# rafifmalikdzaki/Multitask-Bonetumor-yolo

Measured on AMD Instinct MI355X. Metric: images/sec at 640x640 multitask fwd (det+seg+cls) + decode/NMS/masks, higher is better.
Workload: dtype bf16; 1 GPU; configs[1]: batch-16/GPU 640x640 multitask inference (ConvNeXt-T + C2f-BiFPN + Detect/Segment/cls) + decode + per-image NMS(top-100) + mask assembly; random-init weights; batch_per_gpu=16, img=640, parallelism=dp1 (batch sharded, no data-path collective)

## Files before the change

include/mtbt_hip.h:

```cpp
#ifndef MTBT_HIP_H
#define MTBT_HIP_H

#include <stdint.h>

#ifdef __cplusplus
extern "C" {
#endif

#define MTBT_OK 0
#define MTBT_EINVAL (-1)
#define MTBT_EALIGN (-2)
#define MTBT_ELAUNCH (-3)
#define MTBT_EWORKSPACE (-4)

#define MTBT_F32 0
#define MTBT_BF16 1
#define MTBT_F16 2

#define MTBT_ACT_NONE 0
#define MTBT_ACT_SILU 1
#define MTBT_ACT_ELU 2
#define MTBT_ACT_GELU 3
#define MTBT_ACT_DSILU 5
#define MTBT_ACT_DELU 6
// ... 39 lines not shown
  int64_t colsum_ws_bytes;
} mtbt_conv_args;

int mtbt_conv2d_nhwc(const mtbt_conv_args* a, void* stream);
int64_t mtbt_conv_colsum_workspace_bytes(int64_t pixels , int K, int with_squares);
int mtbt_conv_colsum_layout(const mtbt_conv_args* a, int64_t* rows, int32_t* pitch);
int mtbt_conv_kernel_choice(const mtbt_conv_args* a, int32_t* choice);

int mtbt_conv2d_nhwc_batch(const mtbt_conv_args* calls, int n, void* stream);
int mtbt_conv_batch_kernel_choice(const mtbt_conv_args* calls, int n, int32_t* choice);

int mtbt_stem_conv4x4_ln(const float* x, const float* w, const float* bias, const float* ln_w,
                         const float* ln_b, float ln_eps, void* y, int N, int H, int W, int Cout,
                         int out_dtype, void* stream);

int mtbt_dwconv_nhwc(const void* x, const void* w, const float* bias, const float* ln_w,
                     const float* ln_b, float ln_eps, const float* scale, const float* shift, int act,
                     void* y, int N, int H, int W, int C, int ksize, int dtype, void* stream);
int mtbt_dwconv3x3_mult_nhwc(const void* x, const void* w, const float* scale, const float* shift, int act, void* y,
                             int N, int H, int W, int C, int M, int dtype, void* stream);
int mtbt_dwconv_kernel_choice(int N, int H, int W, int C, int ksize, int ln, int act, int dtype, int32_t* choice);
int mtbt_dwconv3x3_mult_kernel_choice(int N, int H, int W, int C, int M, int act, int dtype, int32_t* choice);

int mtbt_layernorm_nhwc(const void* x, const float* w, const float* b, float eps, void* y,
                        int64_t pixels, int C, int dtype, void* stream);

typedef struct mtbt_fuse_args {
  const void* x[3];
  float wgt[3];
  int32_t resample[3];
// ... 691 lines not shown
```

multitask_bonetumor_yolo_amd/_lib.py:

```python
import ctypes as C
import os

_HERE = os.path.dirname(os.path.abspath(__file__))
LIB_PATH = os.path.join(_HERE, "csrc", "libmtbt_hip.so")

ABI_VERSION = 5
F32, BF16, F16 = 0, 1, 2
ACT_NONE, ACT_SILU, ACT_ELU, ACT_GELU, ACT_GELU_POLY, ACT_DSILU, ACT_DELU, ACT_DGELU, ACT_DGELU_POLY = 0, 1, 2, 3, 4, 5, 6, 7, 8
OUT_NHWC, OUT_CONVT2X2 = 0, 1
RES_ID, RES_UP_BILINEAR, RES_DOWN_MEAN, RES_UP_NEAREST, RES_MAXPOOL = 0, 1, 2, 3, 4
CONFUSION_MAX_NC = 64
WARP_CHUNK = 32
WARP_LIN_MAX, WARP_OFF_MAX = 1 << 26, 1 << 47
COPY_PASTE_CHUNK = 8
COPY_PASTE_MAX_ENTRIES = 16

ERRORS = {-1: "MTBT_EINVAL (bad argument / unsupported shape)", -2: "MTBT_EALIGN (misaligned pointer or stride)",
          -3: "MTBT_ELAUNCH (kernel launch failed)", -4: "MTBT_EWORKSPACE (workspace too small)"}


class ConvArgs(C.Structure):
    _fields_ = [
        ("x", C.c_void_p), ("w", C.c_void_p), ("y", C.c_void_p), ("scale", C.c_void_p), ("shift", C.c_void_p),
        ("res", C.c_void_p),
# ... 448 lines not shown
```

multitask_bonetumor_yolo_amd/csrc/dwconv.hip:

```cpp
#include "common.h"
#include "dwconv_args.h"

static int dw_dispatch(const DwArgs& a, int dtype, hipStream_t s) {
  if (dtype == MTBT_BF16) return mtbt_dw_run_bf16(a, s);
  if (dtype == MTBT_F16) return mtbt_dw_run_f16(a, s);
  if (dtype == MTBT_F32) return mtbt_dw_run_f32(a, s);
  return MTBT_EINVAL;
}

static int dw_check_shape(int N, int H, int W, int C, int ksize, int act) {
  if (N <= 0 || H <= 0 || W <= 0 || C <= 0 || C % 8 || C > 768) return MTBT_EINVAL;
  if (ksize != 3 && ksize != 7) return MTBT_EINVAL;
  if (act < 0 || act > MTBT_ACT_DGELU_POLY) return MTBT_EINVAL;
  if ((long)(W + 64) * C * 4 >= 0x7fff0000L || (long)H * W * C >= 0x7fff0000L) return MTBT_EINVAL;
  return MTBT_OK;
}

static int dw_dispatch_mult(const DwArgs& a, int Cx, int dtype, hipStream_t s) {
  if (dtype == MTBT_BF16) return mtbt_dw_run_mult_bf16(a, Cx, s);
  if (dtype == MTBT_F16) return mtbt_dw_run_mult_f16(a, Cx, s);
  if (dtype == MTBT_F32) return mtbt_dw_run_mult_f32(a, Cx, s);
  return MTBT_EINVAL;
}

static int dw_check_shape_mult(int N, int H, int W, int C, int M, int act) {
  if (N <= 0 || H <= 0 || W <= 0 || C <= 0 || C % 128 || (M != 1 && M != 2) || M * C > 768) return MTBT_EINVAL;
  if (act < 0 || act > MTBT_ACT_DGELU_POLY) return MTBT_EINVAL;
  if ((long)(W + 64) * M * C * 4 >= 0x7fff0000L || (long)H * W * M * C >= 0x7fff0000L) return MTBT_EINVAL;
  return MTBT_OK;
}

static int dwconv_entry(const void* x, const void* w, const float* bias, const float* ln_w, const float* ln_b, float ln_eps, const float* scale,
                        const float* shift, int act, void* y, void* raw, const void* res, int N, int H, int W, int C, int ksize, int dtype,
                        void* stream) {
  if (!x || !w || !y) return MTBT_EINVAL;
  if (int rc = dw_check_shape(N, H, W, C, ksize, act)) return rc;
  const bool ln = ln_w != nullptr;
  if (ln && (!ln_b || !bias || res)) return MTBT_EINVAL;
  if (!ln && (!scale || !shift || raw)) return MTBT_EINVAL;
  if (!aligned16(x) || !aligned16(y) || !aligned16(w) || (raw && !aligned16(raw)) || (res && !aligned16(res))) return MTBT_EALIGN;
  DwArgs a{x, w, bias, ln_w, ln_b, ln_eps, scale, shift, act, y, raw, res, N, H, W, C, ksize, nullptr};
  return dw_dispatch(a, dtype, reinterpret_cast<hipStream_t>(stream));
}

extern "C" int mtbt_dwconv_kernel_choice(int N, int H, int W, int C, int ksize, int ln, int act, int dtype, int32_t* choice) {
  if (!choice) return MTBT_EINVAL;
  if (int rc = dw_check_shape(N, H, W, C, ksize, act)) return rc;
  static const float some = 0.f;
  DwArgs a{nullptr, nullptr, nullptr, ln ? &some : nullptr, nullptr, 0.f, nullptr, nullptr, act, nullptr, nullptr, nullptr, N, H, W, C, ksize, choice};
  return dw_dispatch(a, dtype, nullptr);
}

extern "C" int mtbt_dwconv_nhwc(const void* x, const void* w, const float* bias, const float* ln_w, const float* ln_b,
                                float ln_eps, const float* scale, const float* shift, int act, void* y, int N, int H,
                                int W, int C, int ksize, int dtype, void* stream) {
  return dwconv_entry(x, w, bias, ln_w, ln_b, ln_eps, scale, shift, act, y, nullptr, nullptr, N, H, W, C, ksize, dtype, stream);
}

extern "C" int mtbt_dwconv_nhwc_train(const void* x, const void* w, const float* bias, const float* ln_w, const float* ln_b,
                                      float ln_eps, const float* scale, const float* shift, int act, void* y, void* raw, const void* res,
                                      int N, int H, int W, int C, int ksize, int dtype, void* stream) {
  return dwconv_entry(x, w, bias, ln_w, ln_b, ln_eps, scale, shift, act, y, raw, res, N, H, W, C, ksize, dtype, stream);
}

extern "C" int mtbt_dwconv3x3_mult_nhwc(const void* x, const void* w, const float* scale, const float* shift, int act, void* y, int N, int H, int W,
                                        int C, int M, int dtype, void* stream) {
  if (!x || !w || !y || !scale || !shift) return MTBT_EINVAL;
  if (int rc = dw_check_shape_mult(N, H, W, C, M, act)) return rc;
  if (!aligned16(x) || !aligned16(y) || !aligned16(w)) return MTBT_EALIGN;
  DwArgs a{x, w, nullptr, nullptr, nullptr, 0.f, scale, shift, act, y, nullptr, nullptr, N, H, W, M * C, 3, nullptr};
  return dw_dispatch_mult(a, C, dtype, reinterpret_cast<hipStream_t>(stream));
}

extern "C" int mtbt_dwconv3x3_mult_kernel_choice(int N, int H, int W, int C, int M, int act, int dtype, int32_t* choice) {
  if (!choice) return MTBT_EINVAL;
  if (int rc = dw_check_shape_mult(N, H, W, C, M, act)) return rc;
  DwArgs a{nullptr, nullptr, nullptr, nullptr, nullptr, 0.f, nullptr, nullptr, act, nullptr, nullptr, nullptr, N, H, W, M * C, 3, choice};
  return dw_dispatch_mult(a, C, dtype, nullptr);
}
```

multitask_bonetumor_yolo_amd/csrc/dwconv.inc:

```
#include "common.h"
#include "conv_dma.h"
#include "dwconv_args.h"

namespace {

typedef float f32x2 __attribute__((ext_vector_type(2)));
__device__ __forceinline__ f32x2 fma2(f32x2 a, f32x2 b, f32x2 c) { return __builtin_elementwise_fma(a, b, c); }

template <typename T> struct Pair;
template <> struct Pair<float> {
  typedef f32x2 raw_t;
  static __device__ __forceinline__ raw_t ld_raw(const void* p) { return *reinterpret_cast<const f32x2*>(p); }
  static __device__ __forceinline__ f32x2 cvt(raw_t r) { return r; }
  static __device__ __forceinline__ raw_t zero() { return f32x2{0.f, 0.f}; }
  static __device__ __forceinline__ f32x2 ld(const void* p) { return *reinterpret_cast<const f32x2*>(p); }
  static __device__ __forceinline__ void st(float* p, f32x2 v) { *reinterpret_cast<f32x2*>(p) = v; }
};
template <> struct Pair<bf16_t> {
  typedef uint32_t raw_t;
  static __device__ __forceinline__ raw_t ld_raw(const void* p) { return *reinterpret_cast<const uint32_t*>(p); }
  static __device__ __forceinline__ f32x2 cvt(raw_t u) { return f32x2{__uint_as_float(u << 16), __uint_as_float(u & 0xffff0000u)}; }
  static __device__ __forceinline__ raw_t zero() { return 0u; }
  static __device__ __forceinline__ f32x2 ld(const void* p) {
    const uint32_t u = *reinterpret_cast<const uint32_t*>(p);
// ... 99 lines not shown

template <typename T, int TW, bool VARIANTS>
int dw_run_mult(const DwArgs& a, int Cx, hipStream_t s) {
#define DW_M(ACTV, FULLV) launch_dw_mult<T, 4, TW, ACTV, FULLV>(a.x, a.w, a.scale, a.shift, a.act, a.y, a.N, a.H, a.W, a.C, Cx, a.choice, s)
  if constexpr (VARIANTS) {
    const bool full = a.H % 4 == 0 && a.W % TW == 0;
    if (a.act == MTBT_ACT_NONE) return full ? DW_M(MTBT_ACT_NONE, true) : DW_M(MTBT_ACT_NONE, false);
    if (a.act == MTBT_ACT_SILU) return full ? DW_M(MTBT_ACT_SILU, true) : DW_M(MTBT_ACT_SILU, false);
    return full ? DW_M(-1, true) : DW_M(-1, false);
  } else {
    return DW_M(-1, false);
  }
#undef DW_M
}

template <typename T, int KS, bool LN, int TH, int TW, int MAXCH, int XB = 8, int ACT = -1, bool FULL = false, int OCC = 2, bool REGT = (MAXCH == 1)>
int launch_dw(const void* x, const void* w, const float* bias, const float* lnw, const float* lnb, float eps,
              const float* scale, const float* shift, int act, void* y, void* raw, const void* res, int N, int H, int W, int C, int32_t* choice,
              hipStream_t s) {
  constexpr int NT = (TH / 2) * (TW / XB) * 64;
  constexpr int PARTS = CC * (int)sizeof(T) / 16, PXI = 64 / PARTS, IWP = ((TW + KS - 1 + PXI - 1) / PXI) * PXI;
  constexpr int lds_tile = (TH + KS - 1) * IWP * CC * (int)sizeof(T), lds_red = LN ? (NT / 64) * (16 * 64 + 16) * 4 : 0;
  constexpr int lds_taps = REGT ? 0 : ((KS * KS + PXI - 1) / PXI) * 1024;
  constexpr int lds = MAXCH == 1 ? lds_tile + lds_taps + lds_red : (lds_tile + lds_taps > lds_red ? lds_tile + lds_taps : lds_red);
  static_assert(lds <= 160 * 1024, "LDS");
  const long tiles = (long)N * ((H + TH - 1) / TH) * ((W + TW - 1) / TW);
  if (tiles > 0x7fffffffL) return MTBT_EINVAL;
  constexpr int by_waves = (4 * OCC) / (NT / 64) > 0 ? (4 * OCC) / (NT / 64) : 1;
  constexpr int cap = by_waves < 4 ? by_waves : 4;
  const long resident = 256L * (160 * 1024 / lds > cap ? cap : 160 * 1024 / lds);
  long blocks = tiles < resident ? tiles : resident;
  blocks = (blocks + 7) / 8 * 8;
  const int ygrid = MAXCH == 1 ? (C + CC - 1) / CC : 1;
  if (ygrid > 1) { blocks = (blocks / ygrid + 7) / 8 * 8; if (blocks < 8) blocks = 8; }
  if (choice) return dw_report(choice, TH, TW, XB, MAXCH, FULL, ACT, tiles, blocks, ygrid);
  auto kern = dwconv_kernel<T, KS, LN, TH, TW, MAXCH, XB, OCC, REGT, ACT, FULL>;
  if (int rc = mtbt_allow_lds(kern, lds)) return rc;
  hipLaunchKernelGGL(kern, dim3((unsigned)blocks, (unsigned)ygrid), dim3(NT), lds, s, (const T*)x, (const T*)w, bias, lnw, lnb, eps, scale, shift,
                     act, (T*)y, (T*)raw, (const T*)res, N, H, W, C, 0 );
  MTBT_LAUNCH_CHECK();
  return MTBT_OK;
}

template <typename T, int KS, bool LN, int TH, int TW, int ACT, bool FULL>
int dispatch_chunks(const void* x, const void* w, const float* bias, const float* lnw, const float* lnb, float eps,
                    const float* scale, const float* shift, int act, void* y, void* raw, const void* res, int N, int H, int W, int C, bool half,
                    int32_t* choice, hipStream_t s) {
  const int nch = (C + CC - 1) / CC;
  if constexpr (!LN) {
    if constexpr (KS == 7) {
      if (half) return launch_dw<T, KS, LN, TH, TW / 2, 1, 4, ACT, FULL>(x, w, bias, lnw, lnb, eps, scale, shift, act, y, raw, res, N, H, W, C, choice, s);
    }
    return launch_dw<T, KS, LN, TH, TW, 1, 8, ACT, FULL>(x, w, bias, lnw, lnb, eps, scale, shift, act, y, raw, res, N, H, W, C, choice, s);
  } else {
  if (nch <= 1) return launch_dw<T, KS, LN, TH, TW, 1, 8, ACT, FULL>(x, w, bias, lnw, lnb, eps, scale, shift, act, y, raw, res, N, H, W, C, choice, s);
  if (nch <= 2) return launch_dw<T, KS, LN, TH, TW, 2, 8, ACT, FULL>(x, w, bias, lnw, lnb, eps, scale, shift, act, y, raw, res, N, H, W, C, choice, s);
  if (nch <= 3) return launch_dw<T, KS, LN, TH, TW / 2, 3, 4, ACT, FULL>(x, w, bias, lnw, lnb, eps, scale, shift, act, y, raw, res, N, H, W, C, choice, s);
  if (nch <= 6) return launch_dw<T, KS, LN, TH, TW / 2, 6, 4, ACT, FULL, 1>(x, w, bias, lnw, lnb, eps, scale, shift, act, y, raw, res, N, H, W, C, choice, s);
  return MTBT_EINVAL;
  }
}

template <typename T, int TW, bool VARIANTS>
int dw_run(const DwArgs& a, hipStream_t s) {
#define DW_ARGS a.x, a.w, a.bias, a.ln_w, a.ln_b, a.ln_eps, a.scale, a.shift, a.act, a.y, a.raw, a.res, a.N, a.H, a.W, a.C, half, a.choice, s
  const bool ln = a.ln_w != nullptr;
  const bool half = ln ? (a.C + CC - 1) / CC > 2 : (a.ksize == 7 && a.W % TW != 0);
  const int tw = half ? TW / 2 : TW;
  const bool full = VARIANTS && a.H % 4 == 0 && a.W % tw == 0;
#define DW_BY_FULL(KSV, LNV, ACTV) (full ? dispatch_chunks<T, KSV, LNV, 4, TW, ACTV, VARIANTS>(DW_ARGS) : dispatch_chunks<T, KSV, LNV, 4, TW, ACTV, false>(DW_ARGS))
  if (ln) return a.ksize == 7 ? DW_BY_FULL(7, true, 0) : DW_BY_FULL(3, true, 0);
  if (VARIANTS && a.act == MTBT_ACT_NONE) return a.ksize == 7 ? DW_BY_FULL(7, false, (VARIANTS ? MTBT_ACT_NONE : -1)) : DW_BY_FULL(3, false, (VARIANTS ? MTBT_ACT_NONE : -1));
  if (VARIANTS && a.act == MTBT_ACT_SILU) return a.ksize == 7 ? DW_BY_FULL(7, false, (VARIANTS ? MTBT_ACT_SILU : -1)) : DW_BY_FULL(3, false, (VARIANTS ? MTBT_ACT_SILU : -1));
  return a.ksize == 7 ? DW_BY_FULL(7, false, -1) : DW_BY_FULL(3, false, -1);
#undef DW_BY_FULL
#undef DW_ARGS
}

}
```

multitask_bonetumor_yolo_amd/csrc/dwconv_args.h:

```cpp
#pragma once
#include <hip/hip_runtime.h>

struct DwArgs {
  const void* x; const void* w; const float* bias; const float* ln_w; const float* ln_b; float ln_eps;
  const float* scale; const float* shift; int act; void* y; void* raw; const void* res;
  int N, H, W, C, ksize;
  int32_t* choice;
};

int mtbt_dw_run_bf16(const DwArgs& a, hipStream_t s);
int mtbt_dw_run_f16(const DwArgs& a, hipStream_t s);
int mtbt_dw_run_f32(const DwArgs& a, hipStream_t s);
int mtbt_dw_run_mult_bf16(const DwArgs& a, int Cx, hipStream_t s);
int mtbt_dw_run_mult_f16(const DwArgs& a, int Cx, hipStream_t s);
int mtbt_dw_run_mult_f32(const DwArgs& a, int Cx, hipStream_t s);
```

multitask_bonetumor_yolo_amd/csrc/dwconv_body.inc:

```
  const int Cn = C - cg;
  const T* __restrict__ x = x_ + cgx;
  const T* __restrict__ w = w_ + cg;
  T* __restrict__ y = y_ + cg;
  T* __restrict__ raw = raw_ ? raw_ + cg : nullptr;
  const T* res = res_ ? res_ + cg : nullptr;
  const float* __restrict__ bias = bias_ ? bias_ + cg : nullptr;
  const float* __restrict__ lnw = lnw_ ? lnw_ + cg : nullptr;
  const float* __restrict__ lnb = lnb_ ? lnb_ + cg : nullptr;
  const float* __restrict__ scale = scale_ ? scale_ + cg : nullptr;
  const float* __restrict__ shift = shift_ ? shift_ + cg : nullptr;
  constexpr int PAD = KS / 2, YB = 2, SPAN = XB + KS - 1, ROWS = YB + KS - 1;
  constexpr int IH = TH + KS - 1, IW = TW + KS - 1;
  constexpr int ES = (int)sizeof(T), PIXB = CC * ES;
  constexpr int NW = (TH / 2) * (TW / XB);
  constexpr int PARTS = PIXB / 16, PXI = 64 / PARTS, IWP = ((IW + PXI - 1) / PXI) * PXI, SEGS = IWP / PXI;
  constexpr int NDMA = IH * SEGS, DPW = (NDMA + NW - 1) / NW;
  extern __shared__ __attribute__((aligned(16))) char smem[];
  char* tile = smem;
  constexpr int TILEB = IH * IWP * PIXB;
  constexpr int NTI_ = (KS * KS + (64 / (PIXB / 16)) - 1) / (64 / (PIXB / 16));
  constexpr int REDOFF = MAXCH == 1 ? TILEB + (REGT ? 0 : NTI_ * 1024) : 0;
  constexpr int NTI = (KS * KS + PXI - 1) / PXI;

  const int tid = threadIdx.x, lane = tid & 63, wave = tid >> 6;
  const int wave_u = __builtin_amdgcn_readfirstlane(wave);
  const int tiles_x = (W + TW - 1) / TW, tiles_y = (H + TH - 1) / TH;
  const int total = N * tiles_y * tiles_x;
  const int sy = wave / (TW / XB), sx = wave % (TW / XB);
  const int nchunks = (Cn + CC - 1) / CC;
  const unsigned lds0 = (unsigned)(size_t)(__attribute__((address_space(3))) char*)smem;
  const unsigned rowbytes = (unsigned)(W * Cx * ES);
  const unsigned vlane = (unsigned)((lane / PARTS) * Cx * ES + (lane % PARTS) * 16);

  const int xcd = blockIdx.x & 7, slot = blockIdx.x >> 3, per_xcd = (total + 7) >> 3, step = gridDim.x >> 3;
  const int t_end = min(total, (xcd + 1) * per_xcd);

  constexpr bool REGTAPS = REGT;
  f32x2 wr[REGTAPS ? KS * KS : 1];
  if (REGT && lane * 2 < Cn) {
#pragma unroll
    for (int t = 0; t < KS * KS; ++t) wr[REGTAPS ? t : 0] = Pair<T>::ld(w + (unsigned)(t * C + lane * 2));
  }

  f32x2 e0[MAXCH], e1[MAXCH], e2[MAXCH];
#pragma unroll
  for (int k = 0; k < MAXCH; ++k) {
    const int c0 = k * CC + lane * 2;
    e0[k] = e1[k] = e2[k] = f32x2{0.f, 0.f};
    if (c0 < Cn) {
      if constexpr (LN) {
        e0[k] = *reinterpret_cast<const f32x2*>(bias + c0);
// ... 46 lines not shown
#pragma unroll
      for (int a = 0; a < YB; ++a)
#pragma unroll
        for (int i = 0; i < XB; ++i) acc[k][a][i] = f32x2{0.f, 0.f};

    auto chunk = [&](int k) {
      const int cb = k * CC;
      const int cc = min(CC, Cn - cb);
      const bool active = lane * 2 < cc;
      if (MAXCH > 1 || first) {
        lds_barrier();
        stage(tl, cb, MAXCH > 1 || first);
      }
      wait_vm<0>();
      __syncthreads();
      if (active && !(dbg & 1)) {
        const char* lp = tile + ((sy * YB) * IWP + sx * XB) * PIXB + lane * 2 * ES;
        const T* wb = w + cb;
        const unsigned lane2 = (unsigned)lane * 2;
        f32x2 wrow[3][KS], in[2][SPAN];
        auto taps = [&](int ky) {
#pragma unroll
          for (int kx = 0; kx < KS; ++kx) wrow[ky % 3][kx] = Pair<T>::ld(smem + TILEB + (ky * KS + kx) * PIXB + lane2 * ES);
        };
        auto inputs = [&](int r) {
#pragma unroll
          for (int j = 0; j < SPAN; ++j) in[r & 1][j] = Pair<T>::ld(lp + (r * IWP + j) * PIXB);
        };
        if (!REGTAPS) taps(0);
        inputs(0);
#pragma unroll
        for (int r = 0; r < ROWS; ++r) {
          if (!REGTAPS && r + 1 < KS) taps(r + 1);
          if (r + 1 < ROWS) inputs(r + 1);
#pragma unroll
          for (int a = 0; a < YB; ++a) {
            const int ky = r - a;
            if (ky >= 0 && ky < KS) {
#pragma unroll
              for (int kx = 0; kx < KS; ++kx) {
                const f32x2 wv = REGTAPS ? wr[REGTAPS ? ky * KS + kx : 0] : wrow[ky % 3][kx];
#pragma unroll
                for (int i = 0; i < XB; ++i) acc[k][a][i] = fma2(in[r & 1][i + kx], wv, acc[k][a][i]);
              }
            }
          }
          __builtin_amdgcn_sched_barrier(0);
        }
      }
    };
#pragma clang loop unroll(full)
    for (int k = 0; k < MAXCH; ++k)
      if (k < nchunks) chunk(k);
    first = false;
    const int oy0 = ty0 + sy * YB, ox0 = tx0 + sx * XB;
    T* yt = y + (((long)n * H + oy0) * W + ox0) * C;
    const unsigned rowel = (unsigned)(W * C);
    if (dbg & 4) { if (acc[0][0][0].x == 123.f) st_elem<T>(y, 0.f); if (MAXCH == 1) { __syncthreads(); if (tl + step < t_end) stage(tl + step, 0, false); } continue; }
    if (MAXCH == 1) {
      lds_barrier();
      if (tl + step < t_end) stage(tl + step, 0, false);
    }
    if constexpr (LN) {
      if (MAXCH > 1) lds_barrier();
      float* red = reinterpret_cast<float*>(smem + REDOFF) + wave * (16 * 64 + 16);
      float s[16];
#pragma unroll
      for (int pq = 0; pq < 16; ++pq) s[pq] = 0.f;
#pragma unroll
      for (int k = 0; k < MAXCH; ++k) {
        const int c0 = k * CC + lane * 2;
        if (k < nchunks && c0 < Cn) {
          const f32x2 bv = e0[k];
#pragma unroll
          for (int a = 0; a < YB; ++a)
#pragma unroll
            for (int i = 0; i < XB; ++i) {
              acc[k][a][i] += bv;
              s[a * XB + i] += acc[k][a][i].x + acc[k][a][i].y;
            }
        }
      }
      if (raw) {
        T* rt = raw + (((long)n * H + oy0) * W + ox0) * C;
#pragma unroll
        for (int k = 0; k < MAXCH; ++k) {
          const int c0 = k * CC + lane * 2;
          if (k < nchunks && c0 < Cn) {
#pragma unroll
            for (int a = 0; a < YB; ++a) {
              if (!FULL && oy0 + a >= H) continue;
#pragma unroll
              for (int i = 0; i < XB; ++i) {
                if (!FULL && ox0 + i >= W) continue;
                Pair<T>::st(rt + (a * rowel + (unsigned)(i * C + c0)), acc[k][a][i]);
              }
            }
          }
        }
      }
      wave_sum16(s, red, lane);
      const float invC = 1.0f / C;
      float q[16];
#pragma unroll
      for (int pq = 0; pq < 16; ++pq) { s[pq] *= invC; q[pq] = 0.f; }
#pragma unroll
      for (int k = 0; k < MAXCH; ++k) {
        if (k < nchunks && k * CC + lane * 2 < Cn) {
#pragma unroll
          for (int a = 0; a < YB; ++a)
#pragma unroll
            for (int i = 0; i < XB; ++i) {
              const f32x2 d = acc[k][a][i] - s[a * XB + i];
              acc[k][a][i] = d;
              q[a * XB + i] += d.x * d.x + d.y * d.y;
            }
        }
      }
      wave_sum16(q, red, lane);
#pragma unroll
      for (int pq = 0; pq < YB * XB; ++pq) q[pq] = rsqrtf(q[pq] * invC + eps);
#pragma unroll
      for (int k = 0; k < MAXCH; ++k) {
        const int c0 = k * CC + lane * 2;
        if (k < nchunks && c0 < Cn) {
          const f32x2 gw = e1[k], gb = e2[k];
#pragma unroll
          for (int a = 0; a < YB; ++a) {
            if (!FULL && oy0 + a >= H) continue;
#pragma unroll
            for (int i = 0; i < XB; ++i) {
              if (!FULL && ox0 + i >= W) continue;
              Pair<T>::st(yt + (a * rowel + (unsigned)(i * C + c0)), fma2(acc[k][a][i] * q[a * XB + i], gw, gb));
            }
          }
        }
      }
    } else {
#pragma unroll
      for (int k = 0; k < MAXCH; ++k) {
        const int c0 = k * CC + lane * 2;
        if (k < nchunks && c0 < Cn) {
          const f32x2 sc = e0[k], sh = e1[k];
          typename Pair<T>::raw_t rv[YB][XB];
          if (res) {
#pragma unroll
            for (int a = 0; a < YB; ++a)
#pragma unroll
              for (int i = 0; i < XB; ++i) {
                rv[a][i] = Pair<T>::zero();
                if (FULL || (oy0 + a < H && ox0 + i < W))
                  rv[a][i] = Pair<T>::ld_raw(res + (((long)n * H + oy0) * W + ox0) * C + (a * rowel + (unsigned)(i * C + c0)));
// ... 19 lines not shown
```

multitask_bonetumor_yolo_amd/engine.py:

```python
import ctypes as C
import os
from contextlib import contextmanager
from dataclasses import dataclass
from typing import Callable, List, Optional

import torch

from . import _lib as L

TORCH_DTYPE = {L.F32: torch.float32, L.BF16: torch.bfloat16, L.F16: torch.float16}
ESIZE = {L.F32: 4, L.BF16: 2, L.F16: 2}


def code_of(dtype: torch.dtype) -> int:
    if dtype == torch.float32:
        return L.F32
    if dtype == torch.bfloat16:
        return L.BF16
    if dtype == torch.float16:
        return L.F16
    raise ValueError(f"unsupported compute dtype {dtype}: float32 (parity), bfloat16 (throughput) or float16 (inference, BASELINE configs[4])")


@dataclass
# ... 115 lines not shown
    return s


class Plan:
    def __init__(self, device):
        self.lib = L.load()
        self.device = device
        self.pool = Pool(device)
        self.launches: List[Launch] = []
        self.consts = []
        pol = os.environ.get("MTBT_CONV_POLICY")
        self.conv_policy = (0x100 | (int(pol) & 0xff)) if pol is not None else 0
        if os.environ.get("MTBT_DIRECT_TC64"):
            self.conv_policy = 0x100 | ((self.conv_policy & 0xff) if self.conv_policy else 7) | 32
        self.conv_debug = int(os.environ.get("MTBT_CONV_DEBUG", "0"))
        self.reload_env()

    def reload_env(self):
        self.n_lanes = max(1, int(os.environ.get("MTBT_LANES", "4")))
        self.lane_serial = os.environ.get("MTBT_LANE_SERIAL") == "1"
        self.lane_wide_s = float(os.environ.get("MTBT_LANE_WIDE_US", "600")) * 1e-6
        self.lane_window = tuple(int(v) for v in os.environ.get("MTBT_LANE_WINDOW", "0:1000000").split(":"))
        self.__dict__.pop("_sched", None)
        return self

    def run(self, stream: Optional[int] = None, start: int = 0, end: Optional[int] = None, marks=None):
        groups = marks if isinstance(marks, dict) else ({"_": list(marks)} if marks else {})
        unwrap = (lambda r: r) if isinstance(marks, dict) else (lambda r: r.get("_", []))
        sequential = stream is not None or start != 0 or (end is not None and end != len(self.launches)) or self.lanes() <= 1
        if sequential:
# ... 273 lines not shown
        self._io([], [y])

    def dwconv(self, x: Act, w, y: Act, ksize, *, bias=None, lnw=None, lnb=None, eps=0.0, scale=None, shift=None,
               act=L.ACT_NONE, name="dwconv"):
        assert x.dense and y.dense
        p = lambda t: t.data_ptr() if t is not None else None
        if y.C != x.C:
            M = y.C // x.C
            assert ksize == 3 and y.C == M * x.C and bias is None and lnw is None and scale is not None and shift is not None
            args = (x.ptr, w.data_ptr(), p(scale), p(shift), act, y.ptr, x.N, x.H, x.W, x.C, M, x.code)
            n = x.N * x.H * x.W
            self.launches.append(Launch(self.lib.mtbt_dwconv3x3_mult_nhwc, args, name, (x.buf, w, scale, shift, y.buf),
                                        2.0 * n * y.C * 9, 1.0 * n * (x.C + y.C) * ESIZE[x.code]))
            self._io([x, w], [y])
            return
        args = (x.ptr, w.data_ptr(), p(bias), p(lnw), p(lnb), C.c_float(eps), p(scale), p(shift), act, y.ptr,
                x.N, x.H, x.W, x.C, ksize, x.code)
        n = x.N * x.H * x.W * x.C
        self.launches.append(Launch(self.lib.mtbt_dwconv_nhwc, args, name, (x.buf, w, bias, lnw, lnb, scale, shift, y.buf),
                                    2.0 * n * ksize * ksize, 2.0 * n * ESIZE[x.code]))
        self._io([x, w], [y])

    def layernorm(self, x: Act, w, b, eps, y: Act, name="layernorm"):
        assert x.dense and y.dense
        pixels = x.N * x.H * x.W
        args = (x.ptr, w.data_ptr(), b.data_ptr(), C.c_float(eps), y.ptr, pixels, x.C, x.code)
        self.launches.append(Launch(self.lib.mtbt_layernorm_nhwc, args, name, (x.buf, w, b, y.buf), 0.0,
                                    2.0 * pixels * x.C * ESIZE[x.code]))
        self._io([x], [y])

# ... 113 lines not shown
```

Baseline: 2737 images/s.

## Add non-persistent 10x10-tile ring kernel for 7x7 depthwise conv+LN

Adds a new depthwise 7x7 + LayerNorm kernel for bf16/f16 with three channel chunks. It uses 10x10 tiles with one block per tile and double-buffered LDS DMA staging of input and taps, and stages the bias and LN params into LDS. A rule picks it when the ring tile count is small and the persistent kernel would need more tiles than resident slots. The aim is better load balance and less tile-loop tail waste in ConvNeXt stage-3 layers. An env var can force it on or off, and the shared row/LN code is split into include files.

```diff
diff --git a/include/mtbt_hip.h b/include/mtbt_hip.h
--- a/include/mtbt_hip.h
+++ b/include/mtbt_hip.h
@@ -77,6 +77,10 @@
                          const float* ln_b, float ln_eps, void* y, int N, int H, int W, int Cout,
                          int out_dtype, void* stream);
 
+#define MTBT_DW_FORM_RULE 0
+#define MTBT_DW_FORM_NEVER 1
+#define MTBT_DW_FORM_ALWAYS 2
+#define MTBT_DW_FORM(v) ((v) << 8)
 int mtbt_dwconv_nhwc(const void* x, const void* w, const float* bias, const float* ln_w,
                      const float* ln_b, float ln_eps, const float* scale, const float* shift, int act,
                      void* y, int N, int H, int W, int C, int ksize, int dtype, void* stream);
diff --git a/multitask_bonetumor_yolo_amd/_lib.py b/multitask_bonetumor_yolo_amd/_lib.py
--- a/multitask_bonetumor_yolo_amd/_lib.py
+++ b/multitask_bonetumor_yolo_amd/_lib.py
@@ -8,6 +8,7 @@
 F32, BF16, F16 = 0, 1, 2
 ACT_NONE, ACT_SILU, ACT_ELU, ACT_GELU, ACT_GELU_POLY, ACT_DSILU, ACT_DELU, ACT_DGELU, ACT_DGELU_POLY = 0, 1, 2, 3, 4, 5, 6, 7, 8
 OUT_NHWC, OUT_CONVT2X2 = 0, 1
+DW_FORM_RULE, DW_FORM_NEVER, DW_FORM_ALWAYS = 0, 1, 2
 RES_ID, RES_UP_BILINEAR, RES_DOWN_MEAN, RES_UP_NEAREST, RES_MAXPOOL = 0, 1, 2, 3, 4
 CONFUSION_MAX_NC = 64
 WARP_CHUNK = 32
diff --git a/multitask_bonetumor_yolo_amd/csrc/dwconv.hip b/multitask_bonetumor_yolo_amd/csrc/dwconv.hip
--- a/multitask_bonetumor_yolo_amd/csrc/dwconv.hip
+++ b/multitask_bonetumor_yolo_amd/csrc/dwconv.hip
@@ -8,9 +8,13 @@
   return MTBT_EINVAL;
 }
 
-static int dw_check_shape(int N, int H, int W, int C, int ksize, int act) {
+static int dw_check_shape(int N, int H, int W, int C, int ksize, int act, bool ln) {
   if (N <= 0 || H <= 0 || W <= 0 || C <= 0 || C % 8 || C > 768) return MTBT_EINVAL;
   if (ksize != 3 && ksize != 7) return MTBT_EINVAL;
+  if (ln && act >= 0) {
+    if ((act >> 8) > MTBT_DW_FORM_ALWAYS) return MTBT_EINVAL;
+    act &= 0xff;
+  }
   if (act < 0 || act > MTBT_ACT_DGELU_POLY) return MTBT_EINVAL;
   if ((long)(W + 64) * C * 4 >= 0x7fff0000L || (long)H * W * C >= 0x7fff0000L) return MTBT_EINVAL;
   return MTBT_OK;
@@ -34,20 +38,21 @@
                         const float* shift, int act, void* y, void* raw, const void* res, int N, int H, int W, int C, int ksize, int dtype,
                         void* stream) {
   if (!x || !w || !y) return MTBT_EINVAL;
-  if (int rc = dw_check_shape(N, H, W, C, ksize, act)) return rc;
   const bool ln = ln_w != nullptr;
+  if (int rc = dw_check_shape(N, H, W, C, ksize, act, ln)) return rc;
   if (ln && (!ln_b || !bias || res)) return MTBT_EINVAL;
   if (!ln && (!scale || !shift || raw)) return MTBT_EINVAL;
   if (!aligned16(x) || !aligned16(y) || !aligned16(w) || (raw && !aligned16(raw)) || (res && !aligned16(res))) return MTBT_EALIGN;
-  DwArgs a{x, w, bias, ln_w, ln_b, ln_eps, scale, shift, act, y, raw, res, N, H, W, C, ksize, nullptr};
+  DwArgs a{x, w, bias, ln_w, ln_b, ln_eps, scale, shift, ln ? (act & 0xff) : act, y, raw, res, N, H, W, C, ksize, ln ? (act >> 8) : 0, nullptr};
   return dw_dispatch(a, dtype, reinterpret_cast<hipStream_t>(stream));
 }
 
 extern "C" int mtbt_dwconv_kernel_choice(int N, int H, int W, int C, int ksize, int ln, int act, int dtype, int32_t* choice) {
   if (!choice) return MTBT_EINVAL;
-  if (int rc = dw_check_shape(N, H, W, C, ksize, act)) return rc;
+  if (int rc = dw_check_shape(N, H, W, C, ksize, act, ln != 0)) return rc;
   static const float some = 0.f;
-  DwArgs a{nullptr, nullptr, nullptr, ln ? &some : nullptr, nullptr, 0.f, nullptr, nullptr, act, nullptr, nullptr, nullptr, N, H, W, C, ksize, choice};
+  DwArgs a{nullptr, nullptr, nullptr, ln ? &some : nullptr, nullptr, 0.f, nullptr, nullptr, ln ? (act & 0xff) : act, nullptr, nullptr, nullptr, N, H, W, C, ksize,
+           ln ? (act >> 8) : 0, choice};
   return dw_dispatch(a, dtype, nullptr);
 }
 
@@ -68,13 +73,13 @@
   if (!x || !w || !y || !scale || !shift) return MTBT_EINVAL;
   if (int rc = dw_check_shape_mult(N, H, W, C, M, act)) return rc;
   if (!aligned16(x) || !aligned16(y) || !aligned16(w)) return MTBT_EALIGN;
-  DwArgs a{x, w, nullptr, nullptr, nullptr, 0.f, scale, shift, act, y, nullptr, nullptr, N, H, W, M * C, 3, nullptr};
+  DwArgs a{x, w, nullptr, nullptr, nullptr, 0.f, scale, shift, act, y, nullptr, nullptr, N, H, W, M * C, 3, 0, nullptr};
   return dw_dispatch_mult(a, C, dtype, reinterpret_cast<hipStream_t>(stream));
 }
 
 extern "C" int mtbt_dwconv3x3_mult_kernel_choice(int N, int H, int W, int C, int M, int act, int dtype, int32_t* choice) {
   if (!choice) return MTBT_EINVAL;
   if (int rc = dw_check_shape_mult(N, H, W, C, M, act)) return rc;
-  DwArgs a{nullptr, nullptr, nullptr, nullptr, nullptr, 0.f, nullptr, nullptr, act, nullptr, nullptr, nullptr, N, H, W, M * C, 3, choice};
+  DwArgs a{nullptr, nullptr, nullptr, nullptr, nullptr, 0.f, nullptr, nullptr, act, nullptr, nullptr, nullptr, N, H, W, M * C, 3, 0, choice};
   return dw_dispatch_mult(a, C, dtype, nullptr);
 }
diff --git a/multitask_bonetumor_yolo_amd/csrc/dwconv.inc b/multitask_bonetumor_yolo_amd/csrc/dwconv.inc
--- a/multitask_bonetumor_yolo_amd/csrc/dwconv.inc
+++ b/multitask_bonetumor_yolo_amd/csrc/dwconv.inc
@@ -137,21 +137,32 @@
 #undef DW_M
 }
 
+template <typename T, int KS, bool LN, int TH, int TW, int MAXCH, int XB = 8, int OCC = 2, bool REGT = (MAXCH == 1)>
+constexpr int dw_lds() {
+  constexpr int NT = (TH / 2) * (TW / XB) * 64;
+  constexpr int PARTS = CC * (int)sizeof(T) / 16, PXI = 64 / PARTS, IWP = ((TW + KS - 1 + PXI - 1) / PXI) * PXI;
+  constexpr int lds_tile = (TH + KS - 1) * IWP * CC * (int)sizeof(T), lds_red = LN ? (NT / 64) * (16 * 64 + 16) * 4 : 0;
+  constexpr int lds_taps = REGT ? 0 : ((KS * KS + PXI - 1) / PXI) * 1024;
+  return MAXCH == 1 ? lds_tile + lds_taps + lds_red : (lds_tile + lds_taps > lds_red ? lds_tile + lds_taps : lds_red);
+}
+template <typename T, int KS, bool LN, int TH, int TW, int MAXCH, int XB = 8, int OCC = 2, bool REGT = (MAXCH == 1)>
+constexpr long dw_slots() {
+  constexpr int NT = (TH / 2) * (TW / XB) * 64, lds = dw_lds<T, KS, LN, TH, TW, MAXCH, XB, OCC, REGT>();
+  constexpr int by_waves = (4 * OCC) / (NT / 64) > 0 ? (4 * OCC) / (NT / 64) : 1;
+  constexpr int cap = by_waves < 4 ? by_waves : 4;
+  return 256L * (160 * 1024 / lds > cap ? cap : 160 * 1024 / lds);
+}
+
 template <typename T, int KS, bool LN, int TH, int TW, int MAXCH, int XB = 8, int ACT = -1, bool FULL = false, int OCC = 2, bool REGT = (MAXCH == 1)>
 int launch_dw(const void* x, const void* w, const float* bias, const float* lnw, const float* lnb, float eps,
               const float* scale, const float* shift, int act, void* y, void* raw, const void* res, int N, int H, int W, int C, int32_t* choice,
               hipStream_t s) {
   constexpr int NT = (TH / 2) * (TW / XB) * 64;
-  constexpr int PARTS = CC * (int)sizeof(T) / 16, PXI = 64 / PARTS, IWP = ((TW + KS - 1 + PXI - 1) / PXI) * PXI;
-  constexpr int lds_tile = (TH + KS - 1) * IWP * CC * (int)sizeof(T), lds_red = LN ? (NT / 64) * (16 * 64 + 16) * 4 : 0;
-  constexpr int lds_taps = REGT ? 0 : ((KS * KS + PXI - 1) / PXI) * 1024;
-  constexpr int lds = MAXCH == 1 ? lds_tile + lds_taps + lds_red : (lds_tile + lds_taps > lds_red ? lds_tile + lds_taps : lds_red);
+  constexpr int lds = dw_lds<T, KS, LN, TH, TW, MAXCH, XB, OCC, REGT>();
   static_assert(lds <= 160 * 1024, "LDS");
   const long tiles = (long)N * ((H + TH - 1) / TH) * ((W + TW - 1) / TW);
   if (tiles > 0x7fffffffL) return MTBT_EINVAL;
-  constexpr int by_waves = (4 * OCC) / (NT / 64) > 0 ? (4 * OCC) / (NT / 64) : 1;
-  constexpr int cap = by_waves < 4 ? by_waves : 4;
-  const long resident = 256L * (160 * 1024 / lds > cap ? cap : 160 * 1024 / lds);
+  constexpr long resident = dw_slots<T, KS, LN, TH, TW, MAXCH, XB, OCC, REGT>();
   long blocks = tiles < resident ? tiles : resident;
   blocks = (blocks + 7) / 8 * 8;
   const int ygrid = MAXCH == 1 ? (C + CC - 1) / CC : 1;
@@ -165,10 +176,12 @@
   return MTBT_OK;
 }
 
+#include "dwconv_ring.inc"
+
 template <typename T, int KS, bool LN, int TH, int TW, int ACT, bool FULL>
 int dispatch_chunks(const void* x, const void* w, const float* bias, const float* lnw, const float* lnb, float eps,
                     const float* scale, const float* shift, int act, void* y, void* raw, const void* res, int N, int H, int W, int C, bool half,
-                    int32_t* choice, hipStream_t s) {
+                    int form, int32_t* choice, hipStream_t s) {
   const int nch = (C + CC - 1) / CC;
   if constexpr (!LN) {
     if constexpr (KS == 7) {
@@ -178,6 +191,13 @@
   } else {
   if (nch <= 1) return launch_dw<T, KS, LN, TH, TW, 1, 8, ACT, FULL>(x, w, bias, lnw, lnb, eps, scale, shift, act, y, raw, res, N, H, W, C, choice, s);
   if (nch <= 2) return launch_dw<T, KS, LN, TH, TW, 2, 8, ACT, FULL>(x, w, bias, lnw, lnb, eps, scale, shift, act, y, raw, res, N, H, W, C, choice, s);
+  if constexpr (KS == 7 && sizeof(T) == 2) {
+    if (nch == 3 && H % 10 == 0 && W % 10 == 0) {
+      const long ring_tiles = (long)N * (H / 10) * (W / 10), tiles = (long)N * ((H + TH - 1) / TH) * ((W + TW / 2 - 1) / (TW / 2));
+      if (form == MTBT_DW_FORM_ALWAYS || (form == MTBT_DW_FORM_RULE && ring_tiles <= 256 && tiles > dw_slots<T, KS, LN, TH, TW / 2, 3, 4>()))
+        return launch_dw_ring<T, 10, 10, 5, 3, true>(x, w, bias, lnw, lnb, eps, y, raw, N, H, W, C, choice, s);
+    }
+  }
   if (nch <= 3) return launch_dw<T, KS, LN, TH, TW / 2, 3, 4, ACT, FULL>(x, w, bias, lnw, lnb, eps, scale, shift, act, y, raw, res, N, H, W, C, choice, s);
   if (nch <= 6) return launch_dw<T, KS, LN, TH, TW / 2, 6, 4, ACT, FULL, 1>(x, w, bias, lnw, lnb, eps, scale, shift, act, y, raw, res, N, H, W, C, choice, s);
   return MTBT_EINVAL;
@@ -186,7 +206,7 @@
 
 template <typename T, int TW, bool VARIANTS>
 int dw_run(const DwArgs& a, hipStream_t s) {
-#define DW_ARGS a.x, a.w, a.bias, a.ln_w, a.ln_b, a.ln_eps, a.scale, a.shift, a.act, a.y, a.raw, a.res, a.N, a.H, a.W, a.C, half, a.choice, s
+#define DW_ARGS a.x, a.w, a.bias, a.ln_w, a.ln_b, a.ln_eps, a.scale, a.shift, a.act, a.y, a.raw, a.res, a.N, a.H, a.W, a.C, half, a.form, a.choice, s
   const bool ln = a.ln_w != nullptr;
   const bool half = ln ? (a.C + CC - 1) / CC > 2 : (a.ksize == 7 && a.W % TW != 0);
   const int tw = half ? TW / 2 : TW;
diff --git a/multitask_bonetumor_yolo_amd/csrc/dwconv_args.h b/multitask_bonetumor_yolo_amd/csrc/dwconv_args.h
--- a/multitask_bonetumor_yolo_amd/csrc/dwconv_args.h
+++ b/multitask_bonetumor_yolo_amd/csrc/dwconv_args.h
@@ -5,6 +5,7 @@
   const void* x; const void* w; const float* bias; const float* ln_w; const float* ln_b; float ln_eps;
   const float* scale; const float* shift; int act; void* y; void* raw; const void* res;
   int N, H, W, C, ksize;
+  int form;
   int32_t* choice;
 };
 
diff --git a/multitask_bonetumor_yolo_amd/csrc/dwconv_body.inc b/multitask_bonetumor_yolo_amd/csrc/dwconv_body.inc
--- a/multitask_bonetumor_yolo_amd/csrc/dwconv_body.inc
+++ b/multitask_bonetumor_yolo_amd/csrc/dwconv_body.inc
@@ -35,6 +35,7 @@
   const int xcd = blockIdx.x & 7, slot = blockIdx.x >> 3, per_xcd = (total + 7) >> 3, step = gridDim.x >> 3;
   const int t_end = min(total, (xcd + 1) * per_xcd);
 
+  constexpr bool RAWPF = false;
   constexpr bool REGTAPS = REGT;
   f32x2 wr[REGTAPS ? KS * KS : 1];
   if (REGT && lane * 2 < Cn) {
@@ -111,40 +112,7 @@
       }
       wait_vm<0>();
       __syncthreads();
-      if (active && !(dbg & 1)) {
-        const char* lp = tile + ((sy * YB) * IWP + sx * XB) * PIXB + lane * 2 * ES;
-        const T* wb = w + cb;
-        const unsigned lane2 = (unsigned)lane * 2;
-        f32x2 wrow[3][KS], in[2][SPAN];
-        auto taps = [&](int ky) {
-#pragma unroll
-          for (int kx = 0; kx < KS; ++kx) wrow[ky % 3][kx] = Pair<T>::ld(smem + TILEB + (ky * KS + kx) * PIXB + lane2 * ES);
-        };
-        auto inputs = [&](int r) {
-#pragma unroll
-          for (int j = 0; j < SPAN; ++j) in[r & 1][j] = Pair<T>::ld(lp + (r * IWP + j) * PIXB);
-        };
-        if (!REGTAPS) taps(0);
-        inputs(0);
-#pragma unroll
-        for (int r = 0; r < ROWS; ++r) {
-          if (!REGTAPS && r + 1 < KS) taps(r + 1);
-          if (r + 1 < ROWS) inputs(r + 1);
-#pragma unroll
-          for (int a = 0; a < YB; ++a) {
-            const int ky = r - a;
-            if (ky >= 0 && ky < KS) {
-#pragma unroll
-              for (int kx = 0; kx < KS; ++kx) {
-                const f32x2 wv = REGTAPS ? wr[REGTAPS ? ky * KS + kx : 0] : wrow[ky % 3][kx];
-#pragma unroll
-                for (int i = 0; i < XB; ++i) acc[k][a][i] = fma2(in[r & 1][i + kx], wv, acc[k][a][i]);
-              }
-            }
-          }
-          __builtin_amdgcn_sched_barrier(0);
-        }
-      }
+#include "dwconv_rows.inc"
     };
 #pragma clang loop unroll(full)
     for (int k = 0; k < MAXCH; ++k)
@@ -159,80 +127,9 @@
       if (tl + step < t_end) stage(tl + step, 0, false);
     }
     if constexpr (LN) {
-      if (MAXCH > 1) lds_barrier();
-      float* red = reinterpret_cast<float*>(smem + REDOFF) + wave * (16 * 64 + 16);
-      float s[16];
-#pragma unroll
-      for (int pq = 0; pq < 16; ++pq) s[pq] = 0.f;
-#pragma unroll
-      for (int k = 0; k < MAXCH; ++k) {
-        const int c0 = k * CC + lane * 2;
-        if (k < nchunks && c0 < Cn) {
-          const f32x2 bv = e0[k];
-#pragma unroll
-          for (int a = 0; a < YB; ++a)
-#pragma unroll
-            for (int i = 0; i < XB; ++i) {
-              acc[k][a][i] += bv;
-              s[a * XB + i] += acc[k][a][i].x + acc[k][a][i].y;
-            }
-        }
-      }
-      if (raw) {
-        T* rt = raw + (((long)n * H + oy0) * W + ox0) * C;
-#pragma unroll
-        for (int k = 0; k < MAXCH; ++k) {
-          const int c0 = k * CC + lane * 2;
-          if (k < nchunks && c0 < Cn) {
-#pragma unroll
-            for (int a = 0; a < YB; ++a) {
-              if (!FULL && oy0 + a >= H) continue;
-#pragma unroll
-              for (int i = 0; i < XB; ++i) {
-                if (!FULL && ox0 + i >= W) continue;
-                Pair<T>::st(rt + (a * rowel + (unsigned)(i * C + c0)), acc[k][a][i]);
-              }
-            }
-          }
-        }
-      }
-      wave_sum16(s, red, lane);
-      const float invC = 1.0f / C;
-      float q[16];
-#pragma unroll
-      for (int pq = 0; pq < 16; ++pq) { s[pq] *= invC; q[pq] = 0.f; }
-#pragma unroll
-      for (int k = 0; k < MAXCH; ++k) {
-        if (k < nchunks && k * CC + lane * 2 < Cn) {
-#pragma unroll
-          for (int a = 0; a < YB; ++a)
-#pragma unroll
-            for (int i = 0; i < XB; ++i) {
-              const f32x2 d = acc[k][a][i] - s[a * XB + i];
-              acc[k][a][i] = d;
-              q[a * XB + i] += d.x * d.x + d.y * d.y;
-            }
-        }
-      }
-      wave_sum16(q, red, lane);
-#pragma unroll
-      for (int pq = 0; pq < YB * XB; ++pq) q[pq] = rsqrtf(q[pq] * invC + eps);
-#pragma unroll
-      for (int k = 0; k < MAXCH; ++k) {
-        const int c0 = k * CC + lane * 2;
-        if (k < nchunks && c0 < Cn) {
-          const f32x2 gw = e1[k], gb = e2[k];
-#pragma unroll
-          for (int a = 0; a < YB; ++a) {
-            if (!FULL && oy0 + a >= H) continue;
-#pragma unroll
-            for (int i = 0; i < XB; ++i) {
-              if (!FULL && ox0 + i >= W) continue;
-              Pair<T>::st(yt + (a * rowel + (unsigned)(i * C + c0)), fma2(acc[k][a][i] * q[a * XB + i], gw, gb));
-            }
-          }
-        }
-      }
+#define DW_SQNORM(d, a, i) (d.x * d.x + d.y * d.y)
+#include "dwconv_ln.inc"
+#undef DW_SQNORM
     } else {
 #pragma unroll
       for (int k = 0; k < MAXCH; ++k) {
diff --git a/multitask_bonetumor_yolo_amd/csrc/dwconv_ln.inc b/multitask_bonetumor_yolo_amd/csrc/dwconv_ln.inc
--- /dev/null
+++ b/multitask_bonetumor_yolo_amd/csrc/dwconv_ln.inc
@@ -0,0 +1,74 @@
+      if (MAXCH > 1) lds_barrier();
+      float* red = reinterpret_cast<float*>(smem + REDOFF) + wave * (16 * 64 + 16);
+      float s[16];
+#pragma unroll
+      for (int pq = 0; pq < 16; ++pq) s[pq] = 0.f;
+#pragma unroll
+      for (int k = 0; k < MAXCH; ++k) {
+        const int c0 = k * CC + lane * 2;
+        if (k < nchunks && c0 < Cn) {
+          const f32x2 bv = e0[k];
+#pragma unroll
+          for (int a = 0; a < YB; ++a)
+#pragma unroll
+            for (int i = 0; i < XB; ++i) {
+              acc[k][a][i] += bv;
+              s[a * XB + i] += acc[k][a][i].x + acc[k][a][i].y;
+            }
+        }
+      }
+      if (raw) {
+        T* rt = raw + (((long)n * H + oy0) * W + ox0) * C;
+#pragma unroll
+        for (int k = 0; k < MAXCH; ++k) {
+          const int c0 = k * CC + lane * 2;
+          if (k < nchunks && c0 < Cn) {
+#pragma unroll
+            for (int a = 0; a < YB; ++a) {
+              if (!FULL && oy0 + a >= H) continue;
+#pragma unroll
+              for (int i = 0; i < XB; ++i) {
+                if (!FULL && ox0 + i >= W) continue;
+                Pair<T>::st(rt + (a * rowel + (unsigned)(i * C + c0)), acc[k][a][i]);
+              }
+            }
+          }
+        }
+      }
+      wave_sum16(s, red, lane);
+      const float invC = 1.0f / C;
+      float q[16];
+#pragma unroll
+      for (int pq = 0; pq < 16; ++pq) { s[pq] *= invC; q[pq] = 0.f; }
+#pragma unroll
+      for (int k = 0; k < MAXCH; ++k) {
+        if (k < nchunks && k * CC + lane * 2 < Cn) {
+#pragma unroll
+          for (int a = 0; a < YB; ++a)
+#pragma unroll
+            for (int i = 0; i < XB; ++i) {
+              const f32x2 d = acc[k][a][i] - s[a * XB + i];
+              acc[k][a][i] = d;
+              q[a * XB + i] += DW_SQNORM(d, a, i);
+            }
+        }
+      }
+      wave_sum16(q, red, lane);
+#pragma unroll
+      for (int pq = 0; pq < YB * XB; ++pq) q[pq] = rsqrtf(q[pq] * invC + eps);
+#pragma unroll
+      for (int k = 0; k < MAXCH; ++k) {
+        const int c0 = k * CC + lane * 2;
+        if (k < nchunks && c0 < Cn) {
+          const f32x2 gw = e1[k], gb = e2[k];
+#pragma unroll
+          for (int a = 0; a < YB; ++a) {
+            if (!FULL && oy0 + a >= H) continue;
+#pragma unroll
+            for (int i = 0; i < XB; ++i) {
+              if (!FULL && ox0 + i >= W) continue;
+              Pair<T>::st(yt + (a * rowel + (unsigned)(i * C + c0)), fma2(acc[k][a][i] * q[a * XB + i], gw, gb));
+            }
+          }
+        }
+      }
diff --git a/multitask_bonetumor_yolo_amd/csrc/dwconv_ring.inc b/multitask_bonetumor_yolo_amd/csrc/dwconv_ring.inc
--- /dev/null
+++ b/multitask_bonetumor_yolo_amd/csrc/dwconv_ring.inc
@@ -0,0 +1,148 @@
+
+__device__ __forceinline__ float dw_sqnorm_as_persistent(f32x2 d, bool unfused) {
+  float xx = d.x * d.x, yy = d.y * d.y;
+  asm volatile("" : "+v"(xx), "+v"(yy));
+  return unfused ? xx + yy : __builtin_fmaf(d.x, d.x, yy);
+}
+
+template <typename T, int TH, int TW, int XB, int MAXCH, bool FULL>
+__global__ __launch_bounds__((TH / 2) * (TW / XB) * 64) void dwconv_ring_kernel(
+    const T* __restrict__ x, const T* __restrict__ w , const float* __restrict__ bias, const float* __restrict__ lnw,
+    const float* __restrict__ lnb, float eps, T* __restrict__ y, T* __restrict__ raw, int N, int H, int W, int C) {
+  constexpr int KS = 7, PAD = KS / 2, YB = 2, SPAN = XB + KS - 1, ROWS = YB + KS - 1;
+  constexpr int IH = TH + KS - 1, IW = TW + KS - 1;
+  constexpr int ES = (int)sizeof(T), PIXB = CC * ES;
+  constexpr int NW = (TH / 2) * (TW / XB);
+  constexpr int PARTS = PIXB / 16, PXI = 64 / PARTS, IWP = ((IW + PXI - 1) / PXI) * PXI, SEGS = IWP / PXI;
+  constexpr int NDMA = IH * SEGS, NTI = (KS * KS + PXI - 1) / PXI;
+  constexpr int NP = NDMA + NTI, DPW = (NP + NW - 1) / NW;
+  constexpr int TILEB = IH * IWP * PIXB, STAGEB = TILEB + NTI * 1024;
+  constexpr int REDOFF = STAGEB;
+  static_assert(NW * (16 * 64 + 16) * 4 <= STAGEB, "the LayerNorm scratch reuses one stage");
+  constexpr int EOFF = 2 * STAGEB, EVP = (MAXCH * CC * 4 + 1023) / 1024, EVB = EVP * 1024, NE = 3 * EVP;
+  static_assert(2 * DPW + (NE + NW - 1) / NW < 64, "vmcnt is a 6-bit counter");
+  constexpr bool REGTAPS = false, RAWPF = true;
+  constexpr int dbg = 0;
+  const int Cn = C;
+  extern __shared__ __attribute__((aligned(16))) char smem[];
+
+  const int tid = threadIdx.x, lane = tid & 63, wave = tid >> 6;
+  const int wave_u = __builtin_amdgcn_readfirstlane(wave);
+  const int tiles_x = (W + TW - 1) / TW, tiles_y = (H + TH - 1) / TH;
+  const int total = N * tiles_y * tiles_x;
+  const int sy = wave / (TW / XB), sx = wave % (TW / XB);
+  const int nchunks = (C + CC - 1) / CC;
+  const unsigned lds0 = (unsigned)(size_t)(__attribute__((address_space(3))) char*)smem;
+  const unsigned rowbytes = (unsigned)(W * C * ES);
+  const unsigned vlane = (unsigned)((lane / PARTS) * C * ES + (lane % PARTS) * 16);
+
+  const int xcd = blockIdx.x & 7, slot = blockIdx.x >> 3;
+  const int tl = xcd * (total >> 3) + min(xcd, total & 7) + slot;
+  const int tx = tl % tiles_x, ty = (tl / tiles_x) % tiles_y, n = tl / (tiles_x * tiles_y);
+  const int ty0 = ty * TH, tx0 = tx * TW;
+
+  f32x2 wr[1];
+
+#pragma unroll
+  for (int d = 0; d < (NE + NW - 1) / NW; ++d) {
+    const int j = d * NW + wave_u;
+    if (NE % NW != 0 && j >= NE) break;
+    const int v = j / EVP, piece = j - v * EVP;
+    srd_t esrd = make_srd(v == 0 ? bias : v == 1 ? lnw : lnb);
+    esrd.z = __builtin_amdgcn_readfirstlane((unsigned)(C * 4));
+    lds_dma16(esrd, (unsigned)(piece * 1024 + lane * 16), 0, __builtin_amdgcn_readfirstlane(lds0 + EOFF + v * EVB + piece * 1024));
+  }
+
+  const char* xn = reinterpret_cast<const char*>(x + (long)n * H * W * C);
+  auto stage = [&](int k) {
+    const int cb = k * CC;
+    const unsigned dst = lds0 + (unsigned)((k & 1) * STAGEB);
+#pragma unroll
+    for (int d = 0; d < DPW; ++d) {
+      const int j = d * NW + wave_u;
+      if (NP % NW != 0 && j >= NP) break;
+      if (j < NDMA) {
+        const int row = j / SEGS, seg = j - row * SEGS;
+        const int iy = ty0 + row - PAD;
+        const bool rowok = (unsigned)iy < (unsigned)H;
+        srd_t srd = make_srd(xn + (long)(rowok ? iy : 0) * rowbytes);
+        srd.z = __builtin_amdgcn_readfirstlane(rowok ? rowbytes : 0u);
+        srd.w = __builtin_amdgcn_readfirstlane(srd.w);
+        const int ix0 = tx0 - PAD + seg * PXI;
+        const unsigned vo = (unsigned)(ix0 + lane / PARTS) < (unsigned)W ? vlane + (unsigned)((ix0 * C + cb) * ES) : 0x80000000u;
+        lds_dma16(srd, vo, 0, __builtin_amdgcn_readfirstlane(dst + (row * IWP + seg * PXI) * PIXB));
+      } else {
+        const int jt = j - NDMA;
+        srd_t wsrd = make_srd(w);
+        wsrd.z = __builtin_amdgcn_readfirstlane((unsigned)(KS * KS * C * ES));
+        lds_dma16(wsrd, vlane + (unsigned)((jt * PXI * C + cb) * ES), 0, __builtin_amdgcn_readfirstlane(dst + TILEB + jt * 1024));
+      }
+    }
+  };
+  auto wait_older = [&]() {
+    if (NP % NW == 0 || wave_u < NP - (DPW - 1) * NW) wait_vm<DPW>(); else wait_vm<DPW - 1>();
+  };
+
+  stage(0);
+  if (nchunks > 1) stage(1);
+
+  f32x2 acc[MAXCH][YB][XB];
+#pragma unroll
+  for (int k = 0; k < MAXCH; ++k)
+#pragma unroll
+    for (int a = 0; a < YB; ++a)
+#pragma unroll
+      for (int i = 0; i < XB; ++i) acc[k][a][i] = f32x2{0.f, 0.f};
+
+  auto chunk = [&](int k) {
+    const int cb = k * CC;
+    const bool active = lane * 2 < min(CC, Cn - cb);
+    if (k == 0 && nchunks > 1) wait_older(); else wait_vm<0>();
+    lds_barrier();
+    if (k >= 1 && k + 1 < nchunks) stage(k + 1);
+    const char* tile = smem + (k & 1) * STAGEB;
+#include "dwconv_rows.inc"
+  };
+#pragma clang loop unroll(full)
+  for (int k = 0; k < MAXCH; ++k)
+    if (k < nchunks) chunk(k);
+
+  const int oy0 = ty0 + sy * YB, ox0 = tx0 + sx * XB;
+  T* yt = y + (((long)n * H + oy0) * W + ox0) * C;
+  const unsigned rowel = (unsigned)(W * C);
+  f32x2 e0[MAXCH], e1[MAXCH], e2[MAXCH];
+#pragma unroll
+  for (int k = 0; k < MAXCH; ++k) {
+    const char* ev = smem + EOFF + (k * CC + lane * 2) * 4;
+    e0[k] = *reinterpret_cast<const f32x2*>(ev);
+    e1[k] = *reinterpret_cast<const f32x2*>(ev + EVB);
+    e2[k] = *reinterpret_cast<const f32x2*>(ev + 2 * EVB);
+  }
+  {
+#define DW_SQNORM(d, a, i) dw_sqnorm_as_persistent(d, (a) == 1 && ((ox0 + (i)) & 2) != 0)
+#include "dwconv_ln.inc"
+#undef DW_SQNORM
+  }
+}
+
+template <typename T, int TH, int TW, int MAXCH>
+constexpr int dw_ring_lds() {
+  constexpr int PXI = 64 / (CC * (int)sizeof(T) / 16), IWP = ((TW + 6 + PXI - 1) / PXI) * PXI;
+  return 2 * ((TH + 6) * IWP * CC * (int)sizeof(T) + ((49 + PXI - 1) / PXI) * 1024) + 3 * ((MAXCH * CC * 4 + 1023) / 1024) * 1024;
+}
+
+template <typename T, int TH, int TW, int XB, int MAXCH, bool FULL>
+int launch_dw_ring(const void* x, const void* w, const float* bias, const float* lnw, const float* lnb, float eps, void* y, void* raw, int N, int H, int W,
+                   int C, int32_t* choice, hipStream_t s) {
+  constexpr int NT = (TH / 2) * (TW / XB) * 64;
+  constexpr int lds = dw_ring_lds<T, TH, TW, MAXCH>();
+  static_assert(lds <= 160 * 1024, "LDS");
+  const long tiles = (long)N * ((H + TH - 1) / TH) * ((W + TW - 1) / TW);
+  if (tiles > 0x7fffffffL) return MTBT_EINVAL;
+  if (choice) return dw_report(choice, TH, TW, XB, MAXCH, FULL, 0, tiles, tiles, 1);
+  auto kern = dwconv_ring_kernel<T, TH, TW, XB, MAXCH, FULL>;
+  if (int rc = mtbt_allow_lds(kern, lds)) return rc;
+  hipLaunchKernelGGL(kern, dim3((unsigned)tiles), dim3(NT), lds, s, (const T*)x, (const T*)w, bias, lnw, lnb, eps, (T*)y, (T*)raw, N, H, W, C);
+  MTBT_LAUNCH_CHECK();
+  return MTBT_OK;
+}
diff --git a/multitask_bonetumor_yolo_amd/csrc/dwconv_rows.inc b/multitask_bonetumor_yolo_amd/csrc/dwconv_rows.inc
--- /dev/null
+++ b/multitask_bonetumor_yolo_amd/csrc/dwconv_rows.inc
@@ -0,0 +1,47 @@
+      if (active && !(dbg & 1)) {
+        const char* lp = tile + ((sy * YB) * IWP + sx * XB) * PIXB + lane * 2 * ES;
+        const T* wb = w + cb;
+        const unsigned lane2 = (unsigned)lane * 2;
+        f32x2 wrow[3][KS], in[2][SPAN];
+        typename Pair<T>::raw_t wraw[RAWPF ? KS : 1], inraw[RAWPF ? SPAN : 1];
+        auto taps = [&](int ky) {
+#pragma unroll
+          for (int kx = 0; kx < KS; ++kx) {
+            if constexpr (RAWPF) wraw[kx] = Pair<T>::ld_raw(tile + TILEB + (ky * KS + kx) * PIXB + lane2 * ES);
+            else wrow[ky % 3][kx] = Pair<T>::ld(tile + TILEB + (ky * KS + kx) * PIXB + lane2 * ES);
+          }
+        };
+        auto inputs = [&](int r) {
+#pragma unroll
+          for (int j = 0; j < SPAN; ++j) {
+            if constexpr (RAWPF) inraw[j] = Pair<T>::ld_raw(lp + (r * IWP + j) * PIXB);
+            else in[r & 1][j] = Pair<T>::ld(lp + (r * IWP + j) * PIXB);
+          }
+        };
+        if (!REGTAPS) taps(0);
+        inputs(0);
+#pragma unroll
+        for (int r = 0; r < ROWS; ++r) {
+          if constexpr (RAWPF) {
+#pragma unroll
+            for (int kx = 0; kx < KS; ++kx) if (!REGTAPS && r < KS) wrow[r % 3][kx] = Pair<T>::cvt(wraw[kx]);
+#pragma unroll
+            for (int j = 0; j < SPAN; ++j) in[r & 1][j] = Pair<T>::cvt(inraw[j]);
+          }
+          if (!REGTAPS && r + 1 < KS) taps(r + 1);
+          if (r + 1 < ROWS) inputs(r + 1);
+#pragma unroll
+          for (int a = 0; a < YB; ++a) {
+            const int ky = r - a;
+            if (ky >= 0 && ky < KS) {
+#pragma unroll
+              for (int kx = 0; kx < KS; ++kx) {
+                const f32x2 wv = REGTAPS ? wr[REGTAPS ? ky * KS + kx : 0] : wrow[ky % 3][kx];
+#pragma unroll
+                for (int i = 0; i < XB; ++i) acc[k][a][i] = fma2(in[r & 1][i + kx], wv, acc[k][a][i]);
+              }
+            }
+          }
+          __builtin_amdgcn_sched_barrier(0);
+        }
+      }
diff --git a/multitask_bonetumor_yolo_amd/engine.py b/multitask_bonetumor_yolo_amd/engine.py
--- a/multitask_bonetumor_yolo_amd/engine.py
+++ b/multitask_bonetumor_yolo_amd/engine.py
@@ -153,6 +153,7 @@
         if os.environ.get("MTBT_DIRECT_TC64"):
             self.conv_policy = 0x100 | ((self.conv_policy & 0xff) if self.conv_policy else 7) | 32
         self.conv_debug = int(os.environ.get("MTBT_CONV_DEBUG", "0"))
+        self.dw_form = {"0": L.DW_FORM_NEVER, "2": L.DW_FORM_ALWAYS}.get(os.environ.get("MTBT_DW_ROUND"), L.DW_FORM_RULE)
         self.reload_env()
 
     def reload_env(self):
@@ -456,6 +457,8 @@
                                         2.0 * n * y.C * 9, 1.0 * n * (x.C + y.C) * ESIZE[x.code]))
             self._io([x, w], [y])
             return
+        if lnw is not None:
+            act |= self.dw_form << 8
         args = (x.ptr, w.data_ptr(), p(bias), p(lnw), p(lnb), C.c_float(eps), p(scale), p(shift), act, y.ptr,
                 x.N, x.H, x.W, x.C, ksize, x.code)
         n = x.N * x.H * x.W * x.C
```

Measured after the change: 2736 images/s. Within noise of the previous version (-0.0%).
